# allenai/satlas-super-resolution

Measured on AMD Instinct MI355X. Metric: G+D train-step images/sec, higher is better.
Workload: dtype fp32h

## Files before the change

satlas_super_resolution_amd/csrc/conv.hip:

```cpp
#include "conv_epilogue.h"
#include <cstdlib>
#include <cstdio>

namespace {

template <typename T, int KH, int KW, int S, int NT, int MW, int KS>
__device__ __forceinline__ void conv_body(const ssr_conv_desc& d) {
    constexpr int VEC = DT<T>::VEC;
    constexpr int KSTEPS = (KH == 4) ? 1 : 2;
    constexpr int CK = KSTEPS * 2 * VEC, VPR = 2 * KSTEPS, CKP = CK + VEC, BN = 32 * NT;
    constexpr int TH = 2 * MW, TW = 16;
    constexpr int PH = (TH - 1) * S + KH, PW = (TW - 1) * S + KW;
    constexpr int NTHR = 64 * MW * KS;
    constexpr int PVEC = PH * PW * VPR, WVEC = KH * KW * BN * VPR;
    constexpr int NPV = (PVEC + NTHR - 1) / NTHR, NWV = (WVEC + NTHR - 1) / NTHR;
    constexpr int STAGE = (PH * PW + KH * KW * BN) * CKP;
    extern __shared__ __attribute__((aligned(16))) char smem[];
    T* lds = reinterpret_cast<T*>(smem);

    const int tid = threadIdx.x, lane = tid & 63, wave = tid >> 6;
    const int wm = wave % MW, kh = wave / MW;
    const int tiles_x = (d.Gw + TW - 1) / TW, tiles_y = (d.Gh + TH - 1) / TH;
    int b = blockIdx.x;
    const int tx_i = b % tiles_x; b /= tiles_x;
    const int ty_i = b % tiles_y;
    const int n = b / tiles_y;
    const int gy0 = ty_i * TH, gx0 = tx_i * TW;
    const int co0 = blockIdx.y * BN;

    const T* __restrict__ xg = reinterpret_cast<const T*>(d.x.p);
    const T* __restrict__ wg = reinterpret_cast<const T*>(d.w);
    const int upshift = d.up == 2 ? 1 : 0;
    const int LH = d.Hi << upshift, LW = d.Wi << upshift;
// ... 232 lines not shown
    pick_tile(d, nt2, small);
    if (nt2) return small ? launch_conv<T, KH, KW, S, 2, 2, 2>(d, st) : launch_conv<T, KH, KW, S, 2, 4, 2>(d, st);
    return small ? launch_conv<T, KH, KW, S, 1, 2, 2>(d, st) : launch_conv<T, KH, KW, S, 1, 4, 2>(d, st);
}

template <typename T>
int dispatch_geom(const ssr_conv_desc& d, hipStream_t st) {
    if (d.KH == 3 && d.KW == 3 && d.stride == 1) return dispatch_tile<T, 3, 3, 1>(d, st);
    if (d.KH == 4 && d.KW == 4 && d.stride == 2) return dispatch_tile<T, 4, 4, 2>(d, st);
    if (d.KH == 2 && d.KW == 2 && d.stride == 1) return dispatch_tile<T, 2, 2, 1>(d, st);
    return SSR_EUNSUP;
}

typedef __bf16 bf16x2 __attribute__((ext_vector_type(2)));

__device__ __forceinline__ void split4(const u32x4& v, uint2& hi, uint2& lo) {
    const f32x4 f = __builtin_bit_cast(f32x4, v);
    bf16x4 h, l;
#pragma unroll
    for (int k = 0; k < 4; ++k) {
        h[k] = (__bf16)f[k];
        l[k] = (__bf16)(f[k] - (float)h[k]);
    }
    hi = __builtin_bit_cast(uint2, h);
    lo = __builtin_bit_cast(uint2, l);
}

template <int KH, int KW, int NT, int MW, int KS, bool H = false>
__device__ __forceinline__ void conv_body_x3(const ssr_conv_desc& d) {
    constexpr int VEC = 4, CK = 16, VPR = 4, ROWB = 80, BN = 32 * NT, S = 1;
    constexpr int TH = 2 * MW, TW = 16;
    constexpr int PH = (TH - 1) * S + KH, PW = (TW - 1) * S + KW;
    constexpr int NTHR = 64 * MW * KS;
    constexpr int PVEC = PH * PW * VPR, WVEC = KH * KW * BN * VPR;
    constexpr int NPV = (PVEC + NTHR - 1) / NTHR, NWV = (WVEC + NTHR - 1) / NTHR;
    constexpr int STAGE = (PH * PW + KH * KW * BN) * ROWB;
    extern __shared__ __attribute__((aligned(16))) char smem[];

    const int tid = threadIdx.x, lane = tid & 63, wave = tid >> 6;
    const int wm = wave % MW, kh = wave / MW;
    const int tiles_x = (d.Gw + TW - 1) / TW, tiles_y = (d.Gh + TH - 1) / TH;
    int b = blockIdx.x;
    const int tx_i = b % tiles_x; b /= tiles_x;
    const int ty_i = b % tiles_y;
    const int n = b / tiles_y;
    const int gy0 = ty_i * TH, gx0 = tx_i * TW;
    const int co0 = blockIdx.y * BN;

    const float* __restrict__ xg = reinterpret_cast<const float*>(d.x.p);
    const float* __restrict__ wg = reinterpret_cast<const float*>(d.w);
    const float* __restrict__ x2g = reinterpret_cast<const float*>(d.x2.p);
    const int upshift = d.up == 2 ? 1 : 0;
    const int LH = d.Hi << upshift, LW = d.Wi << upshift;
    const int Ktot = d.Cin + d.Cin2;
    const int nchunks = (Ktot + CK - 1) / CK;
    const size_t wchunk = (size_t)KH * KW * d.CoutPad * CK;

    int pgo[NPV], pgo2[NPV], plo[NPV], pch[NPV];
    int wgo[NWV], wlo[NWV];
#pragma unroll
    for (int q = 0; q < NPV; ++q) {
        const int v = tid + q * NTHR;
        const int pix = v / VPR, part = v - pix * VPR;
        const int py = pix / PW, px = pix - py * PW;
        const int ly = gy0 + py - d.pad_y, lx = gx0 + px - d.pad_x;
        const bool ok = v < PVEC && ly >= 0 && ly < LH && lx >= 0 && lx < LW;
        pgo[q] = ok ? (int)(((size_t)(n * d.Hi + (ly >> upshift)) * d.Wi + (lx >> upshift)) * d.x.cs + d.x.coff + part * VEC) : -1;
        pgo2[q] = (ok && x2g) ? (int)(((size_t)(n * d.Hi + (ly >> upshift)) * d.Wi + (lx >> upshift)) * d.x2.cs + d.x2.coff + part * VEC)
                              : -1;
        plo[q] = v < PVEC ? pix * ROWB + part * 8 : -1;
        pch[q] = part * VEC;
    }
#pragma unroll
    for (int q = 0; q < NWV; ++q) {
        const int v = tid + q * NTHR;
        const int row = v / VPR, part = v - row * VPR;
        const int tap = row / BN, co = row - tap * BN;
        wgo[q] = v < WVEC ? (tap * d.CoutPad + co0 + co) * CK + part * VEC : -1;
        wlo[q] = (PH * PW + row) * ROWB + part * 16;
    }
    u32x4 rp[NPV], rw[NWV];
    auto load_chunk = [&](int c) {
        const int c0 = c * CK;
#pragma unroll
        for (int q = 0; q < NPV; ++q) {
            u32x4 val = {0u, 0u, 0u, 0u};
            const int k0 = c0 + pch[q];
            if (pgo[q] >= 0) {
                if (k0 < d.Cin) val = *reinterpret_cast<const u32x4*>(xg + (size_t)pgo[q] + c0);
                else if (k0 < Ktot) val = *reinterpret_cast<const u32x4*>(x2g + (size_t)pgo2[q] + (c0 - d.Cin));
            }
            rp[q] = val;
        }
#pragma unroll
        for (int q = 0; q < NWV; ++q)
            if (wgo[q] >= 0) rw[q] = *reinterpret_cast<const u32x4*>(wg + (size_t)c * wchunk + wgo[q]);
    };
    auto store_chunk = [&](int stage) {
        char* base = smem + stage * STAGE;
        uint2 hi, lo;
#pragma unroll
        for (int q = 0; q < NPV; ++q)
            if (plo[q] >= 0) {
                split_f32x4<H>(rp[q], hi, lo);
                *reinterpret_cast<uint2*>(base + plo[q]) = hi;
                *reinterpret_cast<uint2*>(base + plo[q] + 32) = lo;
            }
#pragma unroll
        for (int q = 0; q < NWV; ++q)
// ... 110 lines not shown
    constexpr size_t lds = 2 * stage > red ? 2 * stage : red;
    static_assert(lds <= 160 * 1024, "LDS budget");
    auto kern = H ? conv_h3_kernel<KH, KW, NT, MW, KS> : conv_x3_kernel<KH, KW, NT, MW, KS>;
    static bool attr_done[SSR_MAX_DEVICES] = {};
    const int attr_dev = ssr_device_ordinal();
    if (!attr_done[attr_dev]) {
        hipError_t e = hipFuncSetAttribute(reinterpret_cast<const void*>(kern), hipFuncAttributeMaxDynamicSharedMemorySize, (int)lds);
        if (e != hipSuccess) return (int)e;
        attr_done[attr_dev] = true;
    }
    const int tiles = ((d.Gw + TW - 1) / TW) * ((d.Gh + TH - 1) / TH) * d.N;
    hipLaunchKernelGGL(kern, dim3(tiles, d.CoutPad / BN, 1), dim3(64 * MW * KS), lds, st, d);
    SSR_LAUNCH_CHECK();
    return SSR_OK;
}


#ifdef SSR_PROBE
#define XPROBE(k) do { if (threadIdx.x == 0) g_probe[(blockIdx.y * gridDim.x + blockIdx.x) * 24 + (k)] = __builtin_amdgcn_s_memtime(); } while (0)
#else
#define XPROBE(k)
#endif
constexpr int X3_OOB = 0x7ffffff0;
__device__ __forceinline__ __amdgpu_buffer_rsrc_t x3_rsrc(const void* p, long bytes) {
    return __builtin_amdgcn_make_buffer_rsrc(const_cast<void*>(p), 0, (int)(bytes > 0x7fffff00L ? 0x7fffff00L : bytes), 0x00020000);
}

template <int KH, int KW, int NT, int MW, int KS, int CPS, int PD>
__device__ __forceinline__ void conv_body_x3p(const ssr_conv_desc& d) {
    constexpr int VPR = 4, ROWB = 80, BN = 32 * NT, NTAP = KH * KW;
    constexpr int TH = 2 * MW, TW = 16;
    constexpr int PH = TH - 1 + KH, PW = TW - 1 + KW;
    constexpr int NTHR = 64 * MW * KS;
    constexpr int PV1 = PH * PW * VPR, WV1 = NTAP * BN * VPR;
    constexpr int PVEC = CPS * PV1, WVEC = CPS * WV1;
    constexpr int NPV = (PVEC + NTHR - 1) / NTHR, NWV = (WVEC + NTHR - 1) / NTHR;
    constexpr int SUB = (PH * PW + NTAP * BN) * ROWB;
    constexpr int STAGE = CPS * SUB;
    extern __shared__ __attribute__((aligned(16))) char smem[];

    XPROBE(0);
    const int tid = threadIdx.x, lane = tid & 63, wave = tid >> 6;
    const int wm = wave % MW, kh = wave / MW;
    const int tiles_x = (d.Gw + TW - 1) / TW, tiles_y = (d.Gh + TH - 1) / TH;
    int b = blockIdx.x;
    const int tx_i = b % tiles_x; b /= tiles_x;
    const int ty_i = b % tiles_y;
    const int n = b / tiles_y;
    const int gy0 = ty_i * TH, gx0 = tx_i * TW;
    const int co0 = blockIdx.y * BN;
    const int upshift = d.up == 2 ? 1 : 0;
    const int LH = d.Hi << upshift, LW = d.Wi << upshift;
    const int Cin = d.Cin, Cin2 = d.Cin2, Ktot = Cin + Cin2;
    const int nchunks = (Ktot + 15) / 16, nst = (nchunks + CPS - 1) / CPS;
    const long xbytes = (long)d.N * d.Hi * d.Wi * 4;
    const void* xp = d.x.p;
    const void* x2p = d.x2.p ? d.x2.p : d.x.p;
    const __amdgpu_buffer_rsrc_t rsw = x3_rsrc(d.w, (long)nchunks * NTAP * d.CoutPad * 64);

    int pgo[NPV], pgo2[NPV], plo[NPV], pk[NPV];
    int wgo[NWV], wlo[NWV], wcc[NWV];
#pragma unroll
    for (int q = 0; q < NPV; ++q) {
        const int v = tid + q * NTHR;
        const int cc = v / PV1, r = v - cc * PV1;
        const int pix = r / VPR, part = r - pix * VPR;
        const int py = pix / PW, px = pix - py * PW;
        const int ly = gy0 + py - d.pad_y, lx = gx0 + px - d.pad_x;
        const bool ok = v < PVEC && ly >= 0 && ly < LH && lx >= 0 && lx < LW;
        const int po = (n * d.Hi + (ly >> upshift)) * d.Wi + (lx >> upshift);
        pgo[q] = ok ? (po * d.x.cs + d.x.coff) * 4 : X3_OOB;
        pgo2[q] = (ok && d.x2.p) ? (po * d.x2.cs + d.x2.coff) * 4 : X3_OOB;
        pk[q] = cc * 16 + part * 4;
        plo[q] = v < PVEC ? cc * SUB + pix * ROWB + part * 8 : -1;
    }
#pragma unroll
    for (int q = 0; q < NWV; ++q) {
        const int v = tid + q * NTHR;
        const int cc = v / WV1, r = v - cc * WV1;
        const int row = r / VPR, part = r - row * VPR;
        const int tap = row / BN, co = row - tap * BN;
        wcc[q] = v < WVEC ? cc : 0x10000;
        wgo[q] = ((cc * NTAP + tap) * d.CoutPad + co0 + co) * 64 + part * 16;
        wlo[q] = v < WVEC ? cc * SUB + (PH * PW + row) * ROWB + part * 16 : -1;
    }
    u32x4 rp[PD][NPV], rw[PD][NWV];
    auto load_stage = [&](int s, auto jc) {
        constexpr int j = decltype(jc)::value;
        const int c0 = s * CPS * 16;
        const bool live = s < nst;
        const bool in_x = c0 < Cin;
        const int cb = in_x ? c0 : c0 - Cin, clim = live ? (in_x ? Cin : Cin2) : 0, cs_bytes = (in_x ? d.x.cs : d.x2.cs);
        const __amdgpu_buffer_rsrc_t rs = x3_rsrc(in_x ? xp : x2p, xbytes * cs_bytes);
#pragma unroll
        for (int q = 0; q < NPV; ++q) {
            const int k = cb + pk[q];
            const int po = in_x ? pgo[q] : pgo2[q];
            rp[j][q] = __builtin_amdgcn_raw_buffer_load_b128(rs, (k < clim && po != X3_OOB) ? po + k * 4 : X3_OOB, 0, 0);
        }
        const int wbase = s * CPS * NTAP * d.CoutPad * 64, cleft = nchunks - s * CPS;
#pragma unroll
        for (int q = 0; q < NWV; ++q)
            rw[j][q] = __builtin_amdgcn_raw_buffer_load_b128(rsw, wcc[q] < cleft ? wgo[q] + wbase : X3_OOB, 0, 0);
    };
    auto store_unit = [&](int buf, auto jc, auto uc) {
        constexpr int j = decltype(jc)::value, u = decltype(uc)::value;
        char* base = smem + buf * STAGE;
        if constexpr (u < NPV) {
            uint2 hi, lo;
            split4(rp[j][u], hi, lo);
            if ((u + 1) * NTHR <= PVEC || plo[u] >= 0) {
                *reinterpret_cast<uint2*>(base + plo[u]) = hi;
                *reinterpret_cast<uint2*>(base + plo[u] + 32) = lo;
            }
        } else {
            constexpr int q = u - NPV;
            if ((q + 1) * NTHR <= WVEC || wlo[q] >= 0) *reinterpret_cast<u32x4*>(base + wlo[q]) = rw[j][q];
        }
    };
    auto store_stage = [&](int buf, auto jc) { static_for<0, NPV + NWV>([&](auto uc) { store_unit(buf, jc, uc); }); };

    f32x16 acc[NT];
#pragma unroll
    for (int t = 0; t < NT; ++t)
#pragma unroll
        for (int r = 0; r < 16; ++r) acc[t][r] = 0.f;
    const int i = lane & 31, g = lane >> 5;
    const int ty = 2 * wm + (i >> 4), tx = i & 15;
    const int a_off = (ty * PW + tx) * ROWB + g * 16;
    const int b_off = (PH * PW + i) * ROWB + g * 16;
    auto contract_h = [&](int buf, auto hc, auto&& between) {
        constexpr int H = decltype(hc)::value;
        constexpr int NITEM = KS == 2 ? (CPS * NTAP + 1 - H) / 2 : CPS * NTAP;
        const char* ab = smem + buf * STAGE + a_off;
        const char* bb = smem + buf * STAGE + b_off;
        bf16x8 fa[2][2], fb[2][NT][2];
        auto issue = [&](auto kc) {
            constexpr int k = decltype(kc)::value, it = KS == 2 ? 2 * k + H : k;
            constexpr int cc = it / NTAP, tap = it % NTAP, ky = tap / KW, kx = tap % KW;
            fa[k & 1][0] = *reinterpret_cast<const bf16x8*>(ab + cc * SUB + (ky * PW + kx) * ROWB);
            fa[k & 1][1] = *reinterpret_cast<const bf16x8*>(ab + cc * SUB + (ky * PW + kx) * ROWB + 32);
#pragma unroll
            for (int t = 0; t < NT; ++t) {
                fb[k & 1][t][0] = *reinterpret_cast<const bf16x8*>(bb + cc * SUB + (tap * BN + t * 32) * ROWB);
// ... 418 lines not shown
```

satlas_super_resolution_amd/csrc/conv_big_x3.hip:

```cpp
#include "common.h"
#include <cstdlib>

namespace {

constexpr int XB_TH = 32, XB_TW = 16;
template <int KT> struct XbT {
    static constexpr int AROW = 80;
    static constexpr int VPP = 4;
    static constexpr int PH = XB_TH + KT - 1, PW = XB_TW + KT - 1, NPIX = PH * PW;
    static constexpr int PATCH = NPIX * AROW;
    static constexpr int WROWS = KT * KT * 64;
    static constexpr int WBYTES = WROWS * AROW;
    static constexpr int BUF = PATCH + WBYTES;
    static constexpr int BIAS = BUF;
    static constexpr int SLABS = BIAS + 256;
    static constexpr int LDS = SLABS + 4 * 32 * 272;
    static constexpr int NPV = (NPIX * VPP + 255) / 256;
    static constexpr int NWV = (WROWS * VPP + 255) / 256;
    static constexpr int NSTEP = KT * KT;
    static constexpr int TAIL = KT == 3 ? 2 : 1;
    static constexpr int LPS = (NPV + NWV + NSTEP - TAIL - 1) / (NSTEP - TAIL);
    static_assert(LDS <= 160 * 1024 && LPS <= 6, "LDS budget / load slots of a step");
};

#define XB_BAR() asm volatile("s_waitcnt lgkmcnt(0)\n\ts_barrier" ::: "memory")
#ifdef SSR_PROBE
#define XB_T() (__builtin_amdgcn_s_memtime())
#define XB_ACC(k, t0) do { const unsigned long long t1_ = XB_T(); xb_t[k] += t1_ - (t0); (t0) = t1_; } while (0)
#else
#define XB_T() 0ull
#define XB_ACC(k, t0) do { } while (0)
#endif
constexpr int XB_OOB = 0x7ffffff0;
constexpr int XB_SLAB_PITCH = 272, XB_SLAB = 32 * XB_SLAB_PITCH;
__device__ __forceinline__ __amdgpu_buffer_rsrc_t xb_rsrc(const void* p, long bytes) {
    return __builtin_amdgcn_make_buffer_rsrc(const_cast<void*>(p), 0, (int)(bytes > 0x7fffff00L ? 0x7fffff00L : (bytes < 0 ? 0 : bytes)), 0x00020000);
}
template <int KT>
__device__ __forceinline__ void xb_pixel(int w, int m, int s, int& row, int& col) {
    row = 8 * w + 2 * m + (s >> 4);
    col = s < 16 ? s : ((s + 32 - (XB_TW + KT - 1)) & 15);
}
__device__ __forceinline__ void xb_split4(const u32x4& v, uint2& hi, uint2& lo) {
    const f32x4 f = __builtin_bit_cast(f32x4, v);
    bf16x4 h, l;
#pragma unroll
    for (int k = 0; k < 4; ++k) {
        h[k] = (__bf16)f[k];
        l[k] = (__bf16)(f[k] - (float)h[k]);
    }
// ... 1 lines not shown
    lo = __builtin_bit_cast(uint2, l);
}

template <int KT, bool H = false>
__device__ __forceinline__ void conv_bigx3_body(const ssr_conv_desc& d) {
    using T = XbT<KT>;
    constexpr int AROW = T::AROW, VPP = T::VPP, PW = T::PW, NPIX = T::NPIX, PATCH = T::PATCH, NPV = T::NPV, NWV = T::NWV, NSTEP = T::NSTEP;
    extern __shared__ __attribute__((aligned(16))) char smem[];
    const int tid = threadIdx.x, lane = tid & 63, wave = tid >> 6;
    const int i = lane & 31, g = lane >> 5;
    const int tiles_x = (d.Gw + XB_TW - 1) / XB_TW, tiles_y = (d.Gh + XB_TH - 1) / XB_TH;
    const int tpi = tiles_x * tiles_y, G = gridDim.x / tpi;
    const int tp = blockIdx.x % tpi, n0 = blockIdx.x / tpi;
    const int tx_i = tp % tiles_x, ty_i = tp / tiles_x;
    const int nimg = (d.N - n0 + G - 1) / G;
    const int gy0 = ty_i * XB_TH, gx0 = tx_i * XB_TW;
    const int co0 = blockIdx.y * 64;
    const int upshift = d.up == 2 ? 1 : 0;
    const int LH = d.Hi << upshift, LW = d.Wi << upshift;
    const int nchunks = (d.Cin + 15) / 16;
    const int wchunk = KT * KT * d.CoutPad * 64;
    const int T_ = nimg * nchunks;
    const int ximg = d.Hi * d.Wi * d.x.cs * 4, oimg = d.Ho * d.Wo;

    unsigned long long xb_t[8] = {0, 0, 0, 0, 0, 0, 0, 0}, xb_t0 = XB_T();
    const unsigned long long xb_start = xb_t0;
    (void)xb_t; (void)xb_start;
    float* bias_lds = reinterpret_cast<float*>(smem + T::BIAS);
    if (tid < 64) bias_lds[tid] = (d.bias && co0 + tid < d.Cout) ? d.bias[co0 + tid] * (H ? SSR_F32H_WSCALE : 1.f) : 0.f;

    const bool s2d = KT == 2 && d.s2d != 0;
    const int cpc_shift = s2d ? 31 - __builtin_clz((unsigned)(d.Cin >> 6)) : 0;
    const int x_cs = d.x.cs, x_Wi = d.Wi, x_Cin = d.Cin;
    static_assert((T::WROWS * VPP) % 256 == 0, "no partial weight vector");
    const int p4 = tid >> 2, part4 = tid & 3;
    const int plo0 = p4 * AROW + part4 * 8;
    const int wlo0 = PATCH + p4 * AROW + part4 * 16;
    const int wgo0 = (co0 + p4) * 64 + part4 * 16, wstep = d.CoutPad * 64;
    constexpr int PTAIL = NPIX * VPP - (NPV - 1) * 256;
    int pgo[NPV];
    unsigned pmk[KT == 2 ? NPV : 1];
    const int climit = s2d ? 0x7fffffff : x_Cin - (tid % VPP) * 4;
#pragma unroll
    for (int q = 0; q < NPV; ++q) {
        const int v = tid + q * 256;
        const int pix = v / VPP, part = v % VPP;
        const int py = pix / PW, px = pix - py * PW;
        const int ly = gy0 + py - d.pad_y, lx = gx0 + px - d.pad_x;
        if constexpr (KT == 2) {
            if (s2d) {
                const int sy = 2 * ly - 1, sx = 2 * lx - 1;
                const bool y0 = sy >= 0 && sy < d.Hi, y1 = sy + 1 >= 0 && sy + 1 < d.Hi;
                const bool x0 = sx >= 0 && sx < d.Wi, x1 = sx + 1 >= 0 && sx + 1 < d.Wi;
                pmk[q] = v < NPIX * VPP ? (unsigned)(y0 && x0) | (unsigned)(y0 && x1) << 1 | (unsigned)(y1 && x0) << 2 | (unsigned)(y1 && x1) << 3 : 0u;
                pgo[q] = ((sy * d.Wi + sx) * d.x.cs + d.x.coff + part * 4) * 4 + (d.Wi + 1) * d.x.cs * 4;
            } else {
                const bool ok = v < NPIX * VPP && ly >= 0 && ly < LH && lx >= 0 && lx < LW;
                pmk[q] = ok ? 1u : 0u;
                pgo[q] = ok ? (((ly >> upshift) * d.Wi + (lx >> upshift)) * d.x.cs + d.x.coff + part * 4) * 4 : XB_OOB;
            }
        } else {
            const bool ok = v < NPIX * VPP && ly >= 0 && ly < LH && lx >= 0 && lx < LW;
            pgo[q] = ok ? (((ly >> upshift) * d.Wi + (lx >> upshift)) * d.x.cs + d.x.coff + part * 4) * 4 : XB_OOB;
        }
    }
    const long xbias = s2d ? (long)(d.Wi + 1) * d.x.cs * 4 : 0;
    const __amdgpu_buffer_rsrc_t rsx = xb_rsrc(reinterpret_cast<const char*>(d.x.p) - xbias, (long)d.N * ximg + xbias),
                                 rsw = xb_rsrc(d.w, (long)nchunks * wchunk);
    u32x4 rp[NPV], rw[NWV];
    struct LoadPos { int q, c0, xs, ws; };
    auto load_pos = [&](int nn, int c) {
        LoadPos p;
        p.c0 = c * 16;
        if constexpr (KT == 2) {
            p.q = s2d ? c >> cpc_shift : 0;
            p.xs = nn * ximg + (s2d ? (((p.q >> 1) * x_Wi + (p.q & 1)) * x_cs + ((c - (p.q << cpc_shift)) << 4)) * 4 : p.c0 * 4);
        } else {
            p.q = 0;
            p.xs = nn * ximg + p.c0 * 4;
        }
        p.ws = c * wchunk;
        return p;
    };
    auto load_one = [&](const LoadPos& lp, auto jc) {
        constexpr int j = decltype(jc)::value;
        if constexpr (j < NPV) {
            bool ok = lp.c0 < climit;
            if constexpr (KT == 2) ok = ok && ((pmk[j] >> lp.q) & 1u);
            rp[j] = __builtin_amdgcn_raw_buffer_load_b128(rsx, ok ? pgo[j] : XB_OOB, lp.xs, 0);
        } else {
            rw[j - NPV] = __builtin_amdgcn_raw_buffer_load_b128(rsw, wgo0, lp.ws + (j - NPV) * wstep, 0);
        }
    };
    auto load_chunk = [&](int nn, int c) { const LoadPos lp = load_pos(nn, c); static_for<0, NPV + NWV>([&](auto jc) { load_one(lp, jc); }); };
    auto store_chunk = [&]() {
        static_for<0, NPV>([&](auto jc) {
            constexpr int j = decltype(jc)::value;
            uint2 hi, lo;
            split_f32x4<H>(rp[j], hi, lo);
            if (j + 1 < NPV || tid < PTAIL) {
                *reinterpret_cast<uint2*>(smem + plo0 + j * 64 * AROW) = hi;
                *reinterpret_cast<uint2*>(smem + plo0 + j * 64 * AROW + 32) = lo;
            }
        });
        static_for<0, NWV>([&](auto jc) {
            constexpr int j = decltype(jc)::value;
            *reinterpret_cast<u32x4*>(smem + wlo0 + j * 64 * AROW) = rw[j];
        });
    };

    int a_off[4];
#pragma unroll
    for (int m = 0; m < 4; ++m) {
        int row, col;
        xb_pixel<KT>(wave, m, i, row, col);
        a_off[m] = (row * PW + col) * AROW + g * 16;
    }
    const int b_off = PATCH + i * AROW + g * 16;
    const int co_l = 4 * g;

    load_chunk(n0, 0);
    __syncthreads();
    XB_ACC(1, xb_t0);
    f32x16 acc[4][2];
    auto acc_init = [&]() {
#pragma unroll
        for (int t = 0; t < 2; ++t)
#pragma unroll
            for (int q4 = 0; q4 < 4; ++q4) {
                const f32x4 bq = *reinterpret_cast<const f32x4*>(bias_lds + t * 32 + 8 * q4 + co_l);
#pragma unroll
                for (int e = 0; e < 4; ++e)
#pragma unroll
// ... 275 lines not shown
```

satlas_super_resolution_amd/csrc/conv_x3c.hip:

```cpp
#include "conv_x3r_core.h"
#include <cstdio>

#ifdef SSR_PROBE
#define CPROBE(cond, k) do { if (cond) g_probe[blockIdx.x * 32 + (k)] = __builtin_amdgcn_s_memtime(); } while (0)
#else
#define CPROBE(cond, k)
#endif

namespace {

constexpr int XC_MAXN = 4;
constexpr int XC_MAXCH = 16;
constexpr int XC_NS = 6;
constexpr int XC_RING = XC_NS * XR_SUB;
constexpr int XC_RED = 16 * XR_SLOT;
constexpr int XC_CTL = XC_RING + XC_RED;
constexpr int XC_LDS = XC_CTL + 256;
static_assert(XC_LDS <= 160 * 1024, "LDS budget");
constexpr int XC_STATE_HDR = 64;
constexpr int XC_POLL_MAX = 1 << 20;

struct ssr_chain_args {
    ssr_conv_desc d[XC_MAXN];
    int32_t n;
// ... 5 lines not shown
};

typedef __attribute__((address_space(1))) unsigned int gu32;
typedef __attribute__((address_space(1))) unsigned char gu8;

template <int EP>
__global__ __launch_bounds__(XR_NTHR) void conv_x3c_kernel(const ssr_chain_args a) {
    using T = XrT<1, 1>;
    constexpr int WR = T::WR, TPS = T::TPS, SPT = 4 / TPS, NSUB = 3 * SPT, NSETS = T::NSETS, PD = NSETS - 1;
    static_assert(WR == 6 && NSUB * 2 % NSETS == 0, "item-parity unrolling");
    extern __shared__ __attribute__((aligned(16))) char smem[];
    int* ctl = reinterpret_cast<int*>(smem + XC_CTL);
    const int ctl_addr = (int)(size_t)(__attribute__((address_space(3))) char*)(smem + XC_CTL);
    const int tid = threadIdx.x, lane = tid & 63, wave = __builtin_amdgcn_readfirstlane(tid >> 6);
    if (tid < 9) ctl[tid] = 0;
    if (tid == 64) {
        ctl[9] = (int)atomicAdd(a.state, 1u);
        ctl[10] = (int)(__hip_atomic_load(a.state + 2, __ATOMIC_RELAXED, __HIP_MEMORY_SCOPE_AGENT) % 255u) + 1;
    }
    __syncthreads();
    const int ticket = __builtin_amdgcn_readfirstlane(ctl[9]);
    const unsigned eb = (unsigned)__builtin_amdgcn_readfirstlane(ctl[10]);
    const int tiles_x = a.tiles_x, tiles = a.tiles_x * a.tiles_y;
    const int n = ticket / tiles, tix = ticket - n * tiles;
    const int ty_i = tix / tiles_x, tx_i = tix - ty_i * tiles_x;
    const int gy0 = ty_i * 8, gx0 = tx_i * 16;
    const int nconv = a.n;
    const int flag_off = XC_STATE_HDR + (n * tiles + tix) * 16;
    CPROBE(tid == 0, 0);

    if (wave >= XR_NMFMA) {
        const int pw = wave - XR_NMFMA;
        const int pt = tid - 64 * XR_NMFMA;
        const int part = pt & 3, p4 = pt >> 2;
        const ssr_conv_desc& d0 = a.d[0];
        int ppix[XR_NPV];
#pragma unroll
        for (int q = 0; q < XR_NPV; ++q) {
            const int pix = p4 + 64 * q;
            const int py = pix / XR_PW, px = pix - py * XR_PW;
            const int ly = gy0 + py - 1, lx = gx0 + px - 1;
            const bool okp = pix < XR_NPIX && ly >= 0 && ly < d0.Hi && lx >= 0 && lx < d0.Wi;
            ppix[q] = okp ? (n * d0.Hi + ly) * d0.Wi + lx : -1;
        }
        const int plo0 = p4 * XR_ROWB + part * 8;
        const long xbytes = (long)d0.N * d0.Hi * d0.Wi * 4;
        const __amdgpu_buffer_rsrc_t rs_state = xr_rsrc(a.state, (long)XC_STATE_HDR + (long)d0.N * tiles * 16);
        int total = 0;
        for (int ci = 0; ci < nconv; ++ci) total += a.nch[ci];
        int seen = -1;
        int nb_off;
        {
            const int l = lane < 9 ? lane : 4;
            int nty = ty_i + l / 3 - 1, ntx = tx_i + l % 3 - 1;
            if (nty < 0 || nty >= a.tiles_y || ntx < 0 || ntx >= tiles_x) { nty = ty_i; ntx = tx_i; }
            nb_off = XC_STATE_HDR + (n * tiles + nty * tiles_x + ntx) * 16;
        }
        auto wait_published = [&](int dep) {
            const unsigned want = eb * 0x01010101u;
            int spin = 0;
            for (; spin < XC_POLL_MAX; ++spin) {
                const unsigned v = (unsigned)__builtin_amdgcn_raw_buffer_load_b32(rs_state, nb_off + dep * 4, 0, 16);
                if (__builtin_amdgcn_ballot_w64(v != want) == 0) break;
                __builtin_amdgcn_s_sleep(8);
            }
            if (spin == XC_POLL_MAX) __builtin_trap();
            seen = dep;
// ... 19 lines not shown
            const int cb = in_x ? c0 : c0 - Cin, clim = live ? (in_x ? Cin : Cin2) : 0;
            const ssr_view& vw = (in_x || !d.x2.p) ? d.x : d.x2;
            const int cs = vw.cs, coff = vw.coff;
            const __amdgpu_buffer_rsrc_t rs = xr_rsrc(vw.p, xbytes * cs);
            const int kk = cb + part * 4;
#pragma unroll
            for (int q = 0; q < XR_NPV; ++q) {
                const int off = (ppix[q] * cs + coff + kk) * 4;
                const bool okl = (kk < clim) & (ppix[q] >= 0);
                rq[j][q] = __builtin_amdgcn_raw_buffer_load_b128(rs, okl ? off : XR_OOB, 0, 16);
            }
        };
        static_for<0, XR_PQ>([&](auto jc) { __builtin_amdgcn_sched_barrier(0); load_job(decltype(jc)::value, jc); __builtin_amdgcn_sched_barrier(0); });
        int cfree = XC_NS;
        for (int k0 = 0; k0 < total; k0 += XR_PQ) {
            static_for<0, XR_PQ>([&](auto jc) {
                constexpr int j = decltype(jc)::value;
                const int k = k0 + j;
                if (k < total) {
                    if (k >= cfree) {
                        int spin = 0;
                        for (; spin < XR_SPIN_MAX; ++spin) {
                            cfree = xr_min4(ctl_addr + 16) + XC_NS;
                            if (k < cfree) break;
                            __builtin_amdgcn_s_sleep(2);
                        }
                        if (spin == XR_SPIN_MAX) __builtin_trap();
                    }
                    char* base = smem + (k % XC_NS) * XR_SUB;
#pragma unroll
                    for (int q = 0; q < XR_NPV; ++q) {
                        uint2 hi, lo;
                        xr_split4(rq[j][q], hi, lo);
                        if (q < XR_NPV - 1 || pt < XR_PV - (XR_NPV - 1) * 256) {
                            *reinterpret_cast<uint2*>(base + plo0 + q * 64 * XR_ROWB) = hi;
                            *reinterpret_cast<uint2*>(base + plo0 + q * 64 * XR_ROWB + 32) = lo;
                        }
                    }
                    asm volatile("" ::: "memory");
                    if (lane == 0) *(xr_lds_int)(uintptr_t)(ctl_addr + 4 * pw) = k + 1;
                    asm volatile("" ::: "memory");
                }
                __builtin_amdgcn_sched_barrier(0);
                load_job(k + XR_PQ, jc);
                __builtin_amdgcn_sched_barrier(0);
            });
        }
    } else {
        const int w = wave;
        const int i = lane & 31, gq = lane >> 5;
        const int a_lane = ((i >> 4) * XR_PW + epi_col<XR_ROT>(i)) * XR_ROWB + gq * 16;
        f32x16 acc[4];
        bf16x8 wf[WR][2];
        bf16x8 af[NSETS][TPS][2];
        int avail = 0;
        auto ensure = [&](int c) {
            if (avail > c) return;
            int spin = 0;
            for (; spin < XR_SPIN_MAX; ++spin) {
                avail = xr_min4(ctl_addr);
                if (avail > c) break;
                __builtin_amdgcn_s_sleep(1);
            }
            if (spin == XR_SPIN_MAX) __builtin_trap();
        };
        auto lds_arrive = [&]() {
            asm volatile("" ::: "memory");
// ... 300 lines not shown
```

satlas_super_resolution_amd/csrc/conv_x3r.hip:

```cpp
#include "conv_x3r_core.h"

#ifdef SSR_PROBE
#define RPROBE(cond, k) do { if (cond) g_probe[(blockIdx.y * gridDim.x + blockIdx.x) * 16 + (k)] = __builtin_amdgcn_s_memtime(); } while (0)
#else
#define RPROBE(cond, k)
#endif

namespace {

template <int NTW, int NU, int EP, int TH = 8, int AM = 0>
__global__ __launch_bounds__((XrT<NTW, NU, TH>::NTHR)) void conv_x3r_kernel(const ssr_conv_desc d) {
    constexpr bool EX = AM == 1, H = AM == 2;
    using T = XrT<NTW, NU, TH>;
    constexpr int NT = NTW, NTT = T::NTT, NMF = T::NMF, BN = T::BN, WR = T::WR, MT = T::MT;
    constexpr int G_NPIX = T::NPIX, G_SUB = T::SUB, G_PV = T::PV, G_NPV = T::NPV;
    extern __shared__ __attribute__((aligned(16))) char smem[];
    int* ctl = reinterpret_cast<int*>(smem + T::CTL);
    const int ctl_addr = (int)(size_t)(__attribute__((address_space(3))) char*)(smem + T::CTL);
    const int tid = threadIdx.x, lane = tid & 63, wave = __builtin_amdgcn_readfirstlane(tid >> 6);
    const int tiles_x = (d.Gw + 15) / 16, tiles_y = (d.Gh + TH - 1) / TH;
    int b = blockIdx.x;
    const int tx_i = b % tiles_x; b /= tiles_x;
    const int ty_i = b % tiles_y;
    const int n = b / tiles_y;
    const int gy0 = ty_i * TH, gx0 = tx_i * 16;
    const int co0 = blockIdx.y * BN;
    const int Cin = d.Cin, Cin2 = d.Cin2;
    const int nchunks = (Cin + Cin2 + 15) / 16;
    const int cout_pad = d.CoutPad;
    const int tapstride = cout_pad * 64, wchunk = 9 * tapstride;
    RPROBE(tid == 0, 0);
    if (tid < 4 + NMF) ctl[tid] = 0;
    __syncthreads();

    f32x16 acc[MT][NT];
#pragma unroll
    for (int t = 0; t < MT; ++t)
#pragma unroll
        for (int u = 0; u < NT; ++u)
#pragma unroll
            for (int r = 0; r < 16; ++r) acc[t][u][r] = 0.f;

    if (wave >= NMF) {
        const int pw = wave - NMF;
        const int pt = tid - 64 * NMF;
#ifdef XR_PRIO
        __builtin_amdgcn_s_setprio(3);
#endif
        const int part = pt & 3, p4 = pt >> 2;
        int ppix[G_NPV];
#pragma unroll
        for (int q = 0; q < G_NPV; ++q) {
            const int pix = p4 + 64 * q;
            const int py = pix / XR_PW, px = pix - py * XR_PW;
            const int ly = gy0 + py - d.pad_y, lx = gx0 + px - d.pad_x;
            const bool okp = pix < G_NPIX && ly >= 0 && ly < d.Hi && lx >= 0 && lx < d.Wi;
            ppix[q] = okp ? (n * d.Hi + ly) * d.Wi + lx : -1;
        }
        const int plo0 = p4 * XR_ROWB + part * 8;
        const long xbytes = (long)d.N * d.Hi * d.Wi * 4;
        const void* xp = d.x.p;
        const void* x2p = d.x2.p ? d.x2.p : d.x.p;
        const int x_cs = d.x.cs, x_coff = d.x.coff, x2_cs = d.x2.p ? d.x2.cs : d.x.cs, x2_coff = d.x2.p ? d.x2.coff : d.x.coff;
        u32x4 rq[XR_PQ][G_NPV];
        auto load_chunk = [&](int c, auto jc) {
            constexpr int j = decltype(jc)::value;
            const bool live = c < nchunks;
            const int c0 = c * 16;
            const bool in_x = c0 < Cin;
            const int cb = in_x ? c0 : c0 - Cin, clim = live ? (in_x ? Cin : Cin2) : 0;
            const int cs = in_x ? x_cs : x2_cs, coff = in_x ? x_coff : x2_coff;
            const __amdgpu_buffer_rsrc_t rs = xr_rsrc(in_x ? xp : x2p, xbytes * cs);
            const int k = cb + part * 4;
#pragma unroll
            for (int q = 0; q < G_NPV; ++q) {
                const int off = (ppix[q] * cs + coff + k) * 4;
                const bool okl = (k < clim) & (ppix[q] >= 0);
#ifdef XR_X_NOXLOAD
                rq[j][q] = u32x4{(unsigned)off, (unsigned)okl, 0u, 0u};
#else
                rq[j][q] = __builtin_amdgcn_raw_buffer_load_b128(rs, okl ? off : XR_OOB, 0, 0);
#endif
            }
        };
        static_for<0, XR_PQ>([&](auto jc) { __builtin_amdgcn_sched_barrier(0); load_chunk(decltype(jc)::value, jc); __builtin_amdgcn_sched_barrier(0); });
        RPROBE(pt == 0, 8);
        int cfree = XR_NS;
        for (int c0 = 0; c0 < nchunks; c0 += XR_PQ) {
            static_for<0, XR_PQ>([&](auto jc) {
                constexpr int j = decltype(jc)::value;
                const int c = c0 + j;
                if (c < nchunks) {
                    if (c >= cfree) {
                        int spin = 0;
                        for (; spin < XR_SPIN_MAX; ++spin) {
                            cfree = xr_minN<NMF>(ctl_addr + 16) + XR_NS;
                            if (c < cfree) break;
                            __builtin_amdgcn_s_sleep(2);
                        }
                        if (spin == XR_SPIN_MAX) __builtin_trap();
                    }
                    char* base = smem + (c % XR_NS) * G_SUB;
#pragma unroll
                    for (int q = 0; q < G_NPV; ++q) {
#ifdef XR_X_NOSTORE
                        asm volatile("" :: "v"(rq[j][q]));
                        continue;
#endif
                        if constexpr (EX) {
                            if (q < G_NPV - 1 || pt < G_PV - (G_NPV - 1) * 256)
                                *reinterpret_cast<u32x4*>(base + p4 * XR_ROWB + part * 16 + q * 64 * XR_ROWB) = rq[j][q];
                        } else {
                            uint2 hi, lo;
                            split_f32x4<H>(rq[j][q], hi, lo);
                            if (q < G_NPV - 1 || pt < G_PV - (G_NPV - 1) * 256) {
                                *reinterpret_cast<uint2*>(base + plo0 + q * 64 * XR_ROWB) = hi;
                                *reinterpret_cast<uint2*>(base + plo0 + q * 64 * XR_ROWB + 32) = lo;
                            }
                        }
                    }
                    asm volatile("" ::: "memory");
                    if (lane == 0) *(xr_lds_int)(uintptr_t)(ctl_addr + 4 * pw) = c + 1;
                    asm volatile("" ::: "memory");
#if defined(XR_PRIO) && XR_PRIO == 1
                    if (c == 0) __builtin_amdgcn_s_setprio(0);
#endif
                }
                __builtin_amdgcn_sched_barrier(0);
                load_chunk(c + XR_PQ, jc);
                __builtin_amdgcn_sched_barrier(0);
            });
        }
        RPROBE(pt == 0, 9);
    } else {
        const int w = wave & 3, ug = wave >> 2;
        const int i = lane & 31, gq = lane >> 5;
        const int a_lane = ((i >> 4) * XR_PW + epi_col<XR_ROT>(i)) * XR_ROWB + gq * 16;
        const __amdgpu_buffer_rsrc_t rsw = xr_rsrc(d.w, (long)nchunks * wchunk);
        const int w_lane = (co0 + 32 * NTW * ug + i) * 64 + gq * 16;
        const int nitems = 3 * nchunks;
        const int nj = nitems > w ? (nitems - w + 3) / 4 : 0;
        const int glast = w + 4 * (nj - 1);
        if (nj == 0) {
            if (lane == 0) *(xr_lds_int)(uintptr_t)(ctl_addr + 16 + 4 * wave) = 0x3fffffff;
        } else {
            bf16x8 wf[WR][NT][2];
            constexpr int TPS = T::TPS, SPT = T::SPT, NSUB = 3 * SPT, NSETS = T::NSETS, PD = NSETS - 1;
            bf16x8 af[NSETS][TPS][2];
// ... 322 lines not shown
```

satlas_super_resolution_amd/csrc/conv_x3r_core.h:

```cpp
#pragma once
#include "conv_epilogue.h"
#include <cstdlib>

namespace {

constexpr int XR_NMFMA = 4, XR_NPROD = 4, XR_NTHR = 64 * (XR_NMFMA + XR_NPROD);
constexpr int XR_ROWB = 80, XR_PH = 10, XR_PW = 18, XR_NPIX = XR_PH * XR_PW;
constexpr int XR_SUB = XR_NPIX * XR_ROWB;
constexpr int XR_NS = 8;
constexpr int XR_RING = XR_NS * XR_SUB;
constexpr int XR_PV = XR_NPIX * 4;
constexpr int XR_NPV = (XR_PV + 255) / 256;
#ifndef XR_PQ_DEPTH
#define XR_PQ_DEPTH 4
#endif
constexpr int XR_PQ = XR_PQ_DEPTH;
constexpr int XR_ROT = 14;
constexpr int XR_OOB = 0x7ffffff0;
constexpr int XR_SPIN_MAX = 1 << 22;
constexpr int XR_TILEB = 2 * XR_PW * XR_ROWB;
constexpr int XR_SLOT = 32 * 32 * 4;

template <int NTW, int NU = 1, int TH = 8> struct XrT {
    static_assert(TH == 8 || TH == 4, "tile height");
    static constexpr int MT = TH / 2;
    static constexpr int PH = TH + 2, NPIX = PH * XR_PW;
    static constexpr int SUB = NPIX * XR_ROWB;
    static constexpr int RING = XR_NS * SUB;
    static constexpr int PV = NPIX * 4, NPV = (PV + 255) / 256;
    static constexpr int NTT = NTW * NU;
    static constexpr int BN = 32 * NTT;
    static constexpr int NMF = 4 * NU;
    static constexpr int NTHR = 64 * (NMF + 4);
    static constexpr int WR = (NTW == 1 && NU == 1) ? 6 : 3;
#ifndef XR_TPS1
#define XR_TPS1 4
#endif
    static constexpr int TPS = (NTW == 1 ? XR_TPS1 : 2) < MT ? (NTW == 1 ? XR_TPS1 : 2) : MT;
    static constexpr int SPT = MT / TPS;
    static constexpr int NSETS = SPT == 1 ? 2 : 3;
    static constexpr int SLOTS = 4 * MT * NTT;
    static constexpr int RED = SLOTS * XR_SLOT;
    static constexpr int CTL = RED > RING ? RED : RING;
    static constexpr int LDS = CTL + 256;
    static_assert(LDS <= 160 * 1024, "LDS budget");
};

__device__ __forceinline__ __amdgpu_buffer_rsrc_t xr_rsrc(const void* p, long bytes) {
    return __builtin_amdgcn_make_buffer_rsrc(const_cast<void*>(p), 0, (int)(bytes > 0x7fffff00L ? 0x7fffff00L : (bytes < 0 ? 0 : bytes)), 0x00020000);
}
__device__ __forceinline__ void xr_split4(const u32x4& v, uint2& hi, uint2& lo) {
    const f32x4 f = __builtin_bit_cast(f32x4, v);
    bf16x4 h, l;
#pragma unroll
    for (int k = 0; k < 4; ++k) {
        h[k] = (__bf16)f[k];
        l[k] = (__bf16)(f[k] - (float)h[k]);
    }
    hi = __builtin_bit_cast(uint2, h);
    lo = __builtin_bit_cast(uint2, l);
}
typedef __attribute__((address_space(3))) int* xr_lds_int;
// ... 83 lines not shown
```

satlas_super_resolution_amd/csrc/wgrad_x3.hip:

```cpp
#include "wgrad_common.h"

namespace {

typedef short wx_s16x4 __attribute__((ext_vector_type(4)));
typedef __attribute__((address_space(3))) wx_s16x4 wx_lds_s16x4;
typedef const __attribute__((address_space(1))) char* wx_gptr;

__device__ __forceinline__ bf16x8 wx_tr_pair(const __bf16* lo, const __bf16* hi) {
    const wx_s16x4 a = __builtin_amdgcn_ds_read_tr16_b64_v4i16((wx_lds_s16x4*)(lo));
    const wx_s16x4 b = __builtin_amdgcn_ds_read_tr16_b64_v4i16((wx_lds_s16x4*)(hi));
    typedef short s16x8 __attribute__((ext_vector_type(8)));
    const s16x8 v = __builtin_shufflevector(a, b, 0, 1, 2, 3, 4, 5, 6, 7);
    return __builtin_bit_cast(bf16x8, v);
}
__device__ __forceinline__ int wx_ld(const int* p) { return __atomic_load_n(p, __ATOMIC_RELAXED); }
__device__ __forceinline__ void wx_sync4(int* cnt, int& phase, int lane) {
    phase += 4;
    if (lane == 0) __atomic_fetch_add(cnt, 1, __ATOMIC_RELAXED);
    while (wx_ld(cnt) < phase) {}
}
__device__ const u32x4 g_wx_zero32[2] = {{0u, 0u, 0u, 0u}, {0u, 0u, 0u, 0u}};

#ifndef WX3_PF
#define WX3_PF 4
// ... 142 lines not shown
                asm volatile("global_load_dwordx4 %0, %1, off offset:16" : "=v"(r[2 * q + 1]) : "v"(src) : "memory");
            }
        };
        auto pass = [&](u32x4 (&r)[2 * NLU]) {
            asm volatile("" : "+v"(r[0]), "+v"(r[1]), "+v"(r[2]), "+v"(r[3]), "+v"(r[4]), "+v"(r[5]), "+v"(r[6]), "+v"(r[7]), "+v"(r[8]), "+v"(r[9]) :: "memory");
            asm volatile("" : "+v"(r[10]), "+v"(r[11]), "+v"(r[12]), "+v"(r[13]), "+v"(r[14]), "+v"(r[15]), "+v"(r[16]), "+v"(r[17]), "+v"(r[18]), "+v"(r[19]) :: "memory");
        };
        auto wait_tile = [&](u32x4 (&r)[2 * NLU]) {
            pass(r);
            asm volatile("s_waitcnt vmcnt(20)" ::: "memory");
            pass(r);
        };
        auto put = [&](int k, int st, u32x4 (&r)[2 * NLU]) {
            wait_tile(r);
            if (k >= NST) {
                for (;;) {
                    u32x4 dn;
                    asm volatile("ds_read_b128 %0, %1\n\ts_waitcnt lgkmcnt(0)" : "=&v"(dn) : "v"((int)(C::CTL + 4 * WXC_DONE)) : "memory");
                    if ((int)min(min(dn[0], dn[1]), min(dn[2], dn[3])) >= k - NST + 1) break;
                }
            }
            char* base = smem + st * C::STAGE;
#pragma unroll
            for (int q = 0; q < NLU; ++q) {
                const f32x4 v0 = __builtin_bit_cast(f32x4, r[2 * q]), v1 = __builtin_bit_cast(f32x4, r[2 * q + 1]);
                bf16x8 h, l;
#pragma unroll
                for (int e = 0; e < 4; ++e) {
                    h[e] = (__bf16)v0[e];
                    l[e] = (__bf16)(v0[e] - (float)h[e]);
                    h[4 + e] = (__bf16)v1[e];
                    l[4 + e] = (__bf16)(v1[e] - (float)h[4 + e]);
                }
                if (q < QDY) {
                    if (wr_dy) {
                        *reinterpret_cast<u32x4*>(base + lo_dy + q * 2048) = __builtin_bit_cast(u32x4, h);
                        *reinterpret_cast<u32x4*>(base + lo_dy + C::DYP + q * 2048) = __builtin_bit_cast(u32x4, l);
                    }
                    if (do_bias) {
#pragma unroll
                        for (int e = 0; e < 4; ++e) {
                            bacc[e] += v0[e];
                            bacc[4 + e] += v1[e];
                        }
                    }
                } else if (lt + (q - QDY) * 256 < C::NXU) {
                    *reinterpret_cast<u32x4*>(base + lo_x + (q - QDY) * 2048) = __builtin_bit_cast(u32x4, h);
                    *reinterpret_cast<u32x4*>(base + lo_x + C::XP + (q - QDY) * 2048) = __builtin_bit_cast(u32x4, l);
                }
            }
            if (lane == 0) asm volatile("ds_add_u32 %0, %1" ::"v"((int)(C::CTL + 4 * (WXC_READY + st))), "v"(1) : "memory");
        };
        const int last = ntile - 1;
        if (ntile > 0) {
            load_tile(0, ra);
            load_tile(min(1, last), rb);
        }
        int k = 0;
        for (; k + 1 < ntile; k += 2) {
            put(k, 0, ra);
            load_tile(min(k + 2, last), ra);
            put(k + 1, 1, rb);
            load_tile(min(k + 3, last), rb);
        }
        if (k < ntile) put(k, 0, ra);
        pass(ra); pass(rb);
// ... 414 lines not shown
```

Before: 1189.

## Permute thread-to-row mapping of LDS staging stores to avoid bank conflicts

Adds a small header with row-permutation functions that shuffle the assignment of threads to patch and weight rows within blocks of eight, and applies it to the staging-store address computation in several conv kernels. The aim is to spread the hi/lo bf16 split stores across LDS banks and cut bank conflicts during tile staging. Tail guards are rewritten to check the permuted row against the patch size, and static_asserts check that the per-thread load count is unchanged. Debug-only NOSTORE probe paths are also added behind macros.

```diff
diff --git a/satlas_super_resolution_amd/csrc/conv.hip b/satlas_super_resolution_amd/csrc/conv.hip
--- a/satlas_super_resolution_amd/csrc/conv.hip
+++ b/satlas_super_resolution_amd/csrc/conv.hip
@@ -1,4 +1,5 @@
 #include "conv_epilogue.h"
+#include "lds_deal.h"
 #include <cstdlib>
 #include <cstdio>
 
@@ -297,8 +298,9 @@
     constexpr int TH = 2 * MW, TW = 16;
     constexpr int PH = (TH - 1) * S + KH, PW = (TW - 1) * S + KW;
     constexpr int NTHR = 64 * MW * KS;
-    constexpr int PVEC = PH * PW * VPR, WVEC = KH * KW * BN * VPR;
+    constexpr int PVEC = lds_deal::pad8(PH * PW) * VPR, WVEC = KH * KW * BN * VPR;
     constexpr int NPV = (PVEC + NTHR - 1) / NTHR, NWV = (WVEC + NTHR - 1) / NTHR;
+    static_assert(NPV == (PH * PW * VPR + NTHR - 1) / NTHR && BN % 8 == 0, "as many loads per thread as the linear map");
     constexpr int STAGE = (PH * PW + KH * KW * BN) * ROWB;
     extern __shared__ __attribute__((aligned(16))) char smem[];
 
@@ -326,20 +328,21 @@
 #pragma unroll
     for (int q = 0; q < NPV; ++q) {
         const int v = tid + q * NTHR;
-        const int pix = v / VPR, part = v - pix * VPR;
+        const int pix = lds_deal::patch_row(v / VPR), part = v % VPR;
+        const bool live = v < PVEC && pix < PH * PW;
         const int py = pix / PW, px = pix - py * PW;
         const int ly = gy0 + py - d.pad_y, lx = gx0 + px - d.pad_x;
-        const bool ok = v < PVEC && ly >= 0 && ly < LH && lx >= 0 && lx < LW;
+        const bool ok = live && ly >= 0 && ly < LH && lx >= 0 && lx < LW;
         pgo[q] = ok ? (int)(((size_t)(n * d.Hi + (ly >> upshift)) * d.Wi + (lx >> upshift)) * d.x.cs + d.x.coff + part * VEC) : -1;
         pgo2[q] = (ok && x2g) ? (int)(((size_t)(n * d.Hi + (ly >> upshift)) * d.Wi + (lx >> upshift)) * d.x2.cs + d.x2.coff + part * VEC)
                               : -1;
-        plo[q] = v < PVEC ? pix * ROWB + part * 8 : -1;
+        plo[q] = live ? pix * ROWB + part * 8 : -1;
         pch[q] = part * VEC;
     }
 #pragma unroll
     for (int q = 0; q < NWV; ++q) {
         const int v = tid + q * NTHR;
-        const int row = v / VPR, part = v - row * VPR;
+        const int row = lds_deal::weight_row(v / VPR), part = v % VPR;
         const int tap = row / BN, co = row - tap * BN;
         wgo[q] = v < WVEC ? (tap * d.CoutPad + co0 + co) * CK + part * VEC : -1;
         wlo[q] = (PH * PW + row) * ROWB + part * 16;
@@ -516,9 +519,10 @@
     constexpr int TH = 2 * MW, TW = 16;
     constexpr int PH = TH - 1 + KH, PW = TW - 1 + KW;
     constexpr int NTHR = 64 * MW * KS;
-    constexpr int PV1 = PH * PW * VPR, WV1 = NTAP * BN * VPR;
+    constexpr int PV1 = lds_deal::pad8(PH * PW) * VPR, WV1 = NTAP * BN * VPR;
     constexpr int PVEC = CPS * PV1, WVEC = CPS * WV1;
     constexpr int NPV = (PVEC + NTHR - 1) / NTHR, NWV = (WVEC + NTHR - 1) / NTHR;
+    static_assert(NPV == (CPS * PH * PW * VPR + NTHR - 1) / NTHR && BN % 8 == 0, "as many loads per thread as the linear map");
     constexpr int SUB = (PH * PW + NTAP * BN) * ROWB;
     constexpr int STAGE = CPS * SUB;
     extern __shared__ __attribute__((aligned(16))) char smem[];
@@ -548,21 +552,22 @@
     for (int q = 0; q < NPV; ++q) {
         const int v = tid + q * NTHR;
         const int cc = v / PV1, r = v - cc * PV1;
-        const int pix = r / VPR, part = r - pix * VPR;
+        const int pix = lds_deal::patch_row(r / VPR), part = r % VPR;
+        const bool live = v < PVEC && pix < PH * PW;
         const int py = pix / PW, px = pix - py * PW;
         const int ly = gy0 + py - d.pad_y, lx = gx0 + px - d.pad_x;
-        const bool ok = v < PVEC && ly >= 0 && ly < LH && lx >= 0 && lx < LW;
+        const bool ok = live && ly >= 0 && ly < LH && lx >= 0 && lx < LW;
         const int po = (n * d.Hi + (ly >> upshift)) * d.Wi + (lx >> upshift);
         pgo[q] = ok ? (po * d.x.cs + d.x.coff) * 4 : X3_OOB;
         pgo2[q] = (ok && d.x2.p) ? (po * d.x2.cs + d.x2.coff) * 4 : X3_OOB;
         pk[q] = cc * 16 + part * 4;
-        plo[q] = v < PVEC ? cc * SUB + pix * ROWB + part * 8 : -1;
+        plo[q] = live ? cc * SUB + pix * ROWB + part * 8 : -1;
     }
 #pragma unroll
     for (int q = 0; q < NWV; ++q) {
         const int v = tid + q * NTHR;
         const int cc = v / WV1, r = v - cc * WV1;
-        const int row = r / VPR, part = r - row * VPR;
+        const int row = lds_deal::weight_row(r / VPR), part = r % VPR;
         const int tap = row / BN, co = row - tap * BN;
         wcc[q] = v < WVEC ? cc : 0x10000;
         wgo[q] = ((cc * NTAP + tap) * d.CoutPad + co0 + co) * 64 + part * 16;
@@ -593,7 +598,7 @@
         if constexpr (u < NPV) {
             uint2 hi, lo;
             split4(rp[j][u], hi, lo);
-            if ((u + 1) * NTHR <= PVEC || plo[u] >= 0) {
+            if (plo[u] >= 0) {
                 *reinterpret_cast<uint2*>(base + plo[u]) = hi;
                 *reinterpret_cast<uint2*>(base + plo[u] + 32) = lo;
             }
diff --git a/satlas_super_resolution_amd/csrc/conv_big_x3.hip b/satlas_super_resolution_amd/csrc/conv_big_x3.hip
--- a/satlas_super_resolution_amd/csrc/conv_big_x3.hip
+++ b/satlas_super_resolution_amd/csrc/conv_big_x3.hip
@@ -1,4 +1,5 @@
 #include "common.h"
+#include "lds_deal.h"
 #include <cstdlib>
 
 namespace {
@@ -15,7 +16,7 @@
     static constexpr int BIAS = BUF;
     static constexpr int SLABS = BIAS + 256;
     static constexpr int LDS = SLABS + 4 * 32 * 272;
-    static constexpr int NPV = (NPIX * VPP + 255) / 256;
+    static constexpr int NPV = (lds_deal::pad8(NPIX) * VPP + 255) / 256;
     static constexpr int NWV = (WROWS * VPP + 255) / 256;
     static constexpr int NSTEP = KT * KT;
     static constexpr int TAIL = KT == 3 ? 2 : 1;
@@ -83,19 +84,22 @@
     const bool s2d = KT == 2 && d.s2d != 0;
     const int cpc_shift = s2d ? 31 - __builtin_clz((unsigned)(d.Cin >> 6)) : 0;
     const int x_cs = d.x.cs, x_Wi = d.Wi, x_Cin = d.Cin;
-    static_assert((T::WROWS * VPP) % 256 == 0, "no partial weight vector");
-    const int p4 = tid >> 2, part4 = tid & 3;
-    const int plo0 = p4 * AROW + part4 * 8;
-    const int wlo0 = PATCH + p4 * AROW + part4 * 16;
-    const int wgo0 = (co0 + p4) * 64 + part4 * 16, wstep = d.CoutPad * 64;
-    constexpr int PTAIL = NPIX * VPP - (NPV - 1) * 256;
+    constexpr bool DEAL = KT == 3;
+    static_assert((T::WROWS * VPP) % 256 == 0 && T::WROWS % 8 == 0, "no partial weight vector, whole blocks of weight rows");
+    const int part4 = tid & 3;
+    const int prow0 = DEAL ? lds_deal::patch_row(tid >> 2) : tid >> 2, wrow0 = DEAL ? lds_deal::weight_row(tid >> 2) : tid >> 2;
+    const int plo0 = prow0 * AROW + part4 * 8;
+    const int wlo0 = PATCH + wrow0 * AROW + part4 * 16;
+    const int wgo0 = (co0 + wrow0) * 64 + part4 * 16, wstep = d.CoutPad * 64;
+    const bool ptail = prow0 + (NPV - 1) * 64 < NPIX;
+    static_assert((NPV - 1) * 64 <= NPIX, "the rows past the end of the patch belong to the last vector only");
     int pgo[NPV];
     unsigned pmk[KT == 2 ? NPV : 1];
     const int climit = s2d ? 0x7fffffff : x_Cin - (tid % VPP) * 4;
 #pragma unroll
     for (int q = 0; q < NPV; ++q) {
-        const int v = tid + q * 256;
-        const int pix = v / VPP, part = v % VPP;
+        const int pix = prow0 + q * 64, part = part4;
+        const bool live = pix < NPIX;
         const int py = pix / PW, px = pix - py * PW;
         const int ly = gy0 + py - d.pad_y, lx = gx0 + px - d.pad_x;
         if constexpr (KT == 2) {
@@ -103,15 +107,15 @@
                 const int sy = 2 * ly - 1, sx = 2 * lx - 1;
                 const bool y0 = sy >= 0 && sy < d.Hi, y1 = sy + 1 >= 0 && sy + 1 < d.Hi;
                 const bool x0 = sx >= 0 && sx < d.Wi, x1 = sx + 1 >= 0 && sx + 1 < d.Wi;
-                pmk[q] = v < NPIX * VPP ? (unsigned)(y0 && x0) | (unsigned)(y0 && x1) << 1 | (unsigned)(y1 && x0) << 2 | (unsigned)(y1 && x1) << 3 : 0u;
+                pmk[q] = live ? (unsigned)(y0 && x0) | (unsigned)(y0 && x1) << 1 | (unsigned)(y1 && x0) << 2 | (unsigned)(y1 && x1) << 3 : 0u;
                 pgo[q] = ((sy * d.Wi + sx) * d.x.cs + d.x.coff + part * 4) * 4 + (d.Wi + 1) * d.x.cs * 4;
             } else {
-                const bool ok = v < NPIX * VPP && ly >= 0 && ly < LH && lx >= 0 && lx < LW;
+                const bool ok = live && ly >= 0 && ly < LH && lx >= 0 && lx < LW;
                 pmk[q] = ok ? 1u : 0u;
                 pgo[q] = ok ? (((ly >> upshift) * d.Wi + (lx >> upshift)) * d.x.cs + d.x.coff + part * 4) * 4 : XB_OOB;
             }
         } else {
-            const bool ok = v < NPIX * VPP && ly >= 0 && ly < LH && lx >= 0 && lx < LW;
+            const bool ok = live && ly >= 0 && ly < LH && lx >= 0 && lx < LW;
             pgo[q] = ok ? (((ly >> upshift) * d.Wi + (lx >> upshift)) * d.x.cs + d.x.coff + part * 4) * 4 : XB_OOB;
         }
     }
@@ -145,11 +149,25 @@
     };
     auto load_chunk = [&](int nn, int c) { const LoadPos lp = load_pos(nn, c); static_for<0, NPV + NWV>([&](auto jc) { load_one(lp, jc); }); };
     auto store_chunk = [&]() {
+#ifdef XB_X_NOSTORE
         static_for<0, NPV>([&](auto jc) {
             constexpr int j = decltype(jc)::value;
             uint2 hi, lo;
             split_f32x4<H>(rp[j], hi, lo);
-            if (j + 1 < NPV || tid < PTAIL) {
+            asm volatile("" :: "v"(hi.x), "v"(hi.y), "v"(lo.x), "v"(lo.y));
+        });
+        static_for<0, NWV>([&](auto jc) {
+            constexpr int j = decltype(jc)::value;
+            const u32x4 w = rw[j];
+            asm volatile("" :: "v"(w));
+        });
+        return;
+#endif
+        static_for<0, NPV>([&](auto jc) {
+            constexpr int j = decltype(jc)::value;
+            uint2 hi, lo;
+            split_f32x4<H>(rp[j], hi, lo);
+            if (j + 1 < NPV || ptail) {
                 *reinterpret_cast<uint2*>(smem + plo0 + j * 64 * AROW) = hi;
                 *reinterpret_cast<uint2*>(smem + plo0 + j * 64 * AROW + 32) = lo;
             }
diff --git a/satlas_super_resolution_amd/csrc/conv_x3c.hip b/satlas_super_resolution_amd/csrc/conv_x3c.hip
--- a/satlas_super_resolution_amd/csrc/conv_x3c.hip
+++ b/satlas_super_resolution_amd/csrc/conv_x3c.hip
@@ -61,7 +61,8 @@
     if (wave >= XR_NMFMA) {
         const int pw = wave - XR_NMFMA;
         const int pt = tid - 64 * XR_NMFMA;
-        const int part = pt & 3, p4 = pt >> 2;
+        const int part = pt & 3, p4 = lds_deal::patch_row(pt >> 2);
+        const bool ptail = p4 + (XR_NPV - 1) * 64 < XR_NPIX;
         const ssr_conv_desc& d0 = a.d[0];
         int ppix[XR_NPV];
 #pragma unroll
@@ -147,7 +148,7 @@
                     for (int q = 0; q < XR_NPV; ++q) {
                         uint2 hi, lo;
                         xr_split4(rq[j][q], hi, lo);
-                        if (q < XR_NPV - 1 || pt < XR_PV - (XR_NPV - 1) * 256) {
+                        if (q < XR_NPV - 1 || ptail) {
                             *reinterpret_cast<uint2*>(base + plo0 + q * 64 * XR_ROWB) = hi;
                             *reinterpret_cast<uint2*>(base + plo0 + q * 64 * XR_ROWB + 32) = lo;
                         }
diff --git a/satlas_super_resolution_amd/csrc/conv_x3r.hip b/satlas_super_resolution_amd/csrc/conv_x3r.hip
--- a/satlas_super_resolution_amd/csrc/conv_x3r.hip
+++ b/satlas_super_resolution_amd/csrc/conv_x3r.hip
@@ -13,7 +13,7 @@
     constexpr bool EX = AM == 1, H = AM == 2;
     using T = XrT<NTW, NU, TH>;
     constexpr int NT = NTW, NTT = T::NTT, NMF = T::NMF, BN = T::BN, WR = T::WR, MT = T::MT;
-    constexpr int G_NPIX = T::NPIX, G_SUB = T::SUB, G_PV = T::PV, G_NPV = T::NPV;
+    constexpr int G_NPIX = T::NPIX, G_SUB = T::SUB, G_NPV = T::NPV;
     extern __shared__ __attribute__((aligned(16))) char smem[];
     int* ctl = reinterpret_cast<int*>(smem + T::CTL);
     const int ctl_addr = (int)(size_t)(__attribute__((address_space(3))) char*)(smem + T::CTL);
@@ -47,7 +47,8 @@
 #ifdef XR_PRIO
         __builtin_amdgcn_s_setprio(3);
 #endif
-        const int part = pt & 3, p4 = pt >> 2;
+        const int part = pt & 3, p4 = EX ? lds_deal::weight_row(pt >> 2) : lds_deal::patch_row(pt >> 2);
+        const bool ptail = p4 + (G_NPV - 1) * 64 < G_NPIX;
         int ppix[G_NPV];
 #pragma unroll
         for (int q = 0; q < G_NPV; ++q) {
@@ -108,12 +109,12 @@
                         continue;
 #endif
                         if constexpr (EX) {
-                            if (q < G_NPV - 1 || pt < G_PV - (G_NPV - 1) * 256)
+                            if (q < G_NPV - 1 || ptail)
                                 *reinterpret_cast<u32x4*>(base + p4 * XR_ROWB + part * 16 + q * 64 * XR_ROWB) = rq[j][q];
                         } else {
                             uint2 hi, lo;
                             split_f32x4<H>(rq[j][q], hi, lo);
-                            if (q < G_NPV - 1 || pt < G_PV - (G_NPV - 1) * 256) {
+                            if (q < G_NPV - 1 || ptail) {
                                 *reinterpret_cast<uint2*>(base + plo0 + q * 64 * XR_ROWB) = hi;
                                 *reinterpret_cast<uint2*>(base + plo0 + q * 64 * XR_ROWB + 32) = lo;
                             }
diff --git a/satlas_super_resolution_amd/csrc/conv_x3r_core.h b/satlas_super_resolution_amd/csrc/conv_x3r_core.h
--- a/satlas_super_resolution_amd/csrc/conv_x3r_core.h
+++ b/satlas_super_resolution_amd/csrc/conv_x3r_core.h
@@ -1,5 +1,6 @@
 #pragma once
 #include "conv_epilogue.h"
+#include "lds_deal.h"
 #include <cstdlib>
 
 namespace {
@@ -11,6 +12,7 @@
 constexpr int XR_RING = XR_NS * XR_SUB;
 constexpr int XR_PV = XR_NPIX * 4;
 constexpr int XR_NPV = (XR_PV + 255) / 256;
+static_assert(XR_NPV == (lds_deal::pad8(XR_NPIX) * 4 + 255) / 256 && (XR_NPV - 1) * 64 <= XR_NPIX, "whole blocks of 8 pixel slots (lds_deal.h), the slots past the end in the last vector");
 #ifndef XR_PQ_DEPTH
 #define XR_PQ_DEPTH 4
 #endif
@@ -28,6 +30,7 @@
     static constexpr int SUB = NPIX * XR_ROWB;
     static constexpr int RING = XR_NS * SUB;
     static constexpr int PV = NPIX * 4, NPV = (PV + 255) / 256;
+    static_assert(NPV == (lds_deal::pad8(NPIX) * 4 + 255) / 256 && (NPV - 1) * 64 <= NPIX, "whole blocks of 8 pixel slots (lds_deal.h), the slots past the end in the last vector");
     static constexpr int NTT = NTW * NU;
     static constexpr int BN = 32 * NTT;
     static constexpr int NMF = 4 * NU;
diff --git a/satlas_super_resolution_amd/csrc/lds_deal.h b/satlas_super_resolution_amd/csrc/lds_deal.h
--- /dev/null
+++ b/satlas_super_resolution_amd/csrc/lds_deal.h
@@ -0,0 +1,18 @@
+#pragma once
+
+#if defined(__HIPCC__) || defined(__CUDACC__)
+#define LDS_DEAL_FN __host__ __device__ constexpr
+#else
+#define LDS_DEAL_FN constexpr
+#endif
+
+namespace lds_deal {
+
+constexpr int VPR = 4;
+
+LDS_DEAL_FN int pad8(int rows) { return (rows + 7) & ~7; }
+
+LDS_DEAL_FN int patch_row(int s) { return (s & ~7) | ((s & 3) << 1) | ((s >> 2) & 1); }
+LDS_DEAL_FN int weight_row(int s) { return (s & ~7) | ((s >> 1) & 3) | ((s & 1) << 2); }
+
+}
diff --git a/satlas_super_resolution_amd/csrc/wgrad_x3.hip b/satlas_super_resolution_amd/csrc/wgrad_x3.hip
--- a/satlas_super_resolution_amd/csrc/wgrad_x3.hip
+++ b/satlas_super_resolution_amd/csrc/wgrad_x3.hip
@@ -198,6 +198,12 @@
                     h[4 + e] = (__bf16)v1[e];
                     l[4 + e] = (__bf16)(v1[e] - (float)h[4 + e]);
                 }
+#ifdef WX_X_NOSTORE
+                asm volatile("" :: "v"(h), "v"(l), "v"(base));
+                if (q >= QDY || !do_bias) continue;
+                for (int e = 0; e < 4; ++e) { bacc[e] += v0[e]; bacc[4 + e] += v1[e]; }
+                continue;
+#endif
                 if (q < QDY) {
                     if (wr_dy) {
                         *reinterpret_cast<u32x4*>(base + lo_dy + q * 2048) = __builtin_bit_cast(u32x4, h);
```

New measurement: 1194, median of 6. No clear change (+0.4%).
